# laomao0/BIN

Hardware: AMD Instinct MI355X
Metric: interpolated frames/sec at 1280x720 (higher is better)
Workload: dtype f16x3 (fp16 hi+lo pairs = 22-bit significands, 3 MFMA products, f32 accumulate; fp32-class: 1e-6 vs the fp32 reference); 1 GPU; Adobe240 test_blur 1280x720 inference, batch=1 per GPU (6-frame window padded to 768x1344 by the test.py rule), window-sharded; precision=f16x3, streams=1, pipelined_steps=False, four_call_schedule=False, parity=max-abs <= 2e-5 (f16x3) vs the fp32 reference (tests/)

## Files before the change

bin_amd/_lib.py:

```python
import ctypes as C
import os
from functools import partial

from . import build as _build
from .build import BY_NAME, LIB_PATH

RDN_LAYERS = 66
RDN_MAX_LAYERS, RDN_MAX_CONVS = 192, 7
PLAN_KEEP_ACTS, PLAN_NO_FUSE, PLAN_RDB3, PLAN_FUSED_UPNET, PLAN_FUSED_UPNET_TRAIN = 1, 2, 4, 8, 16
PLAN_UPNET_FOLD = 32
BWD_ACCUMULATE = 1
BWD_SAVED_X3 = 2
BWD_FUSED_UPNET = 4
EPI_PLANES, EPI_SHUFFLE, EPI_FINAL, EPI_FINAL_SUBPIX = 0, 1, 2, 4
PROF_WGRAD = 16
LOSS_CHARBONNIER, LOSS_L1_SUM, LOSS_L2_SUM = 0, 1, 2
RDN_LAYOUT_WORDS, RDN_BWD_LAYOUT_WORDS = 16, 24


class BinConvDesc(C.Structure):
    _fields_ = [("N", C.c_int32), ("H", C.c_int32), ("W", C.c_int32), ("ksize", C.c_int32),
                ("cin_chunks", C.c_int32), ("cout", C.c_int32), ("cout_pad", C.c_int32),
                ("nterms", C.c_int32), ("epilogue", C.c_int32), ("relu", C.c_int32),
                ("x_cpg", C.c_int32), ("x_group_stride", C.c_int64), ("n_images", C.c_int32),
                ("reserved", C.c_int32), ("status", C.c_void_p)]


LOSS_MAX_TERMS = 24
CONV_HALF_LAST_CHUNK = 1
CONV_UPNET_FOLD = 2


class BinLossTerms(C.Structure):
    _fields_ = [("x", C.c_void_p * LOSS_MAX_TERMS), ("y", C.c_void_p * LOSS_MAX_TERMS), ("n_terms", C.c_int32)]


class BinLossGrads(C.Structure):
    _fields_ = [("out", C.c_void_p * LOSS_MAX_TERMS), ("term_a", C.c_int32 * LOSS_MAX_TERMS),
                ("term_b", C.c_int32 * LOSS_MAX_TERMS), ("sign_a", C.c_float * LOSS_MAX_TERMS),
                ("sign_b", C.c_float * LOSS_MAX_TERMS), ("n_out", C.c_int32)]


class BinRdnShape(C.Structure):
# ... 356 lines not shown
```

bin_amd/csrc/binhip_fused.h:

```cpp
#pragma once
#include "binhip_conv_common.h"

struct TailKArgs {
    const _Float16 *x_hi, *x_lo;
    const _Float16 *wc_hi, *wc_lo;
    const _Float16 *wl_hi, *wl_lo;
    const float *bc, *bl;
    _Float16 *y_hi, *y_lo;
    _Float16 *o3_hi, *o3_lo;
    unsigned* flags;
    int N, H, W, tiles_x, tiles_y, wt;
#if BINHIP_TIMELINE
    void* tl;
    unsigned tl_launch, tl_base;
#endif
};

int bh_launch_tail_x3(const TailKArgs& a, hipStream_t s);
```

bin_amd/csrc/binhip_fused_x3.hip:

```cpp
#include "binhip_fused.h"
#include <type_traits>

namespace {

struct TX {
    static constexpr int R = 2, NW = 4, TH = 8, PH = 10, PW = 34;
    static constexpr int PP = (PH * PW * 2 + 63) / 64;
    static constexpr int CWP = 9, LWP = 3;
    static constexpr int PATCH_BYTES = PP * 1024;
    static constexpr int WPL = (CWP + LWP) * 1024;
    static constexpr int WBUF_BYTES = 2 * WPL;
    static constexpr int W_OFF = 2 * PATCH_BYTES;
    static constexpr int LDS_BYTES = W_OFF + 2 * WBUF_BYTES;
    static constexpr int NCHUNK = 12;
    static constexpr int NPJ = (PP + NW - 1) / NW;
    static constexpr int TAILW_OFF = W_OFF;
    static_assert(2 * LDS_BYTES <= 160 * 1024, "two workgroups per CU");
};

__device__ __forceinline__ void tx_issue_patch(const TailKArgs& a, char* smem, int c, int pl, int wave, const unsigned* voff,
                                               const ConvTile& t) {
    __amdgpu_buffer_rsrc_t rs = patch_plane(a, c, pl, t);
    char* lds = smem + pl * TX::PATCH_BYTES;
#pragma unroll
    for (int j = 0; j < TX::NPJ; ++j) {
        const int i = wave + TX::NW * j;
        if (i < TX::PP) __builtin_amdgcn_raw_ptr_buffer_load_lds(rs, (lds_void_t*)(lds + i * 1024), 16, voff[j], 0, 0, 0);
    }
}

__device__ __forceinline__ void tx_issue_weights(const TailKArgs& a, char* smem, int c, int buf, int wave, int lane) {
    __amdgpu_buffer_rsrc_t ch = __builtin_amdgcn_make_buffer_rsrc((void*)(a.wc_hi + (long long)c * (9 * 32 * 16)), 0, 9 * 1024, 0x00020000);
    __amdgpu_buffer_rsrc_t cl = __builtin_amdgcn_make_buffer_rsrc((void*)(a.wc_lo + (long long)c * (9 * 32 * 16)), 0, 9 * 1024, 0x00020000);
    __amdgpu_buffer_rsrc_t lh = __builtin_amdgcn_make_buffer_rsrc((void*)(a.wl_hi + (long long)c * (96 * 16)), 0, 3 * 1024, 0x00020000);
    __amdgpu_buffer_rsrc_t ll = __builtin_amdgcn_make_buffer_rsrc((void*)(a.wl_lo + (long long)c * (96 * 16)), 0, 3 * 1024, 0x00020000);
    char* lds = smem + TX::W_OFF + buf * TX::WBUF_BYTES;
    const unsigned v = (unsigned)(lane * 16);
#pragma unroll
    for (int j = 0; j < 6; ++j) {
        const int i = wave + TX::NW * j;
        const int pl = i >= 12 ? 1 : 0;
        const int k = i - 12 * pl;
        const bool lff = k >= TX::CWP;
        const int t = lff ? k - TX::CWP : k;
        __builtin_amdgcn_raw_ptr_buffer_load_lds(pl ? (lff ? ll : cl) : (lff ? lh : ch), (lds_void_t*)(lds + i * 1024), 16, v,
                                                 t * 1024, 0, 0);
    }
}

__device__ __forceinline__ void tx_issue_tailw(const TailKArgs& a, char* smem, int wave, int lane) {
    __amdgpu_buffer_rsrc_t lh = __builtin_amdgcn_make_buffer_rsrc((void*)(a.wl_hi + (long long)12 * (96 * 16)), 0, 6 * 1024, 0x00020000);
    __amdgpu_buffer_rsrc_t ll = __builtin_amdgcn_make_buffer_rsrc((void*)(a.wl_lo + (long long)12 * (96 * 16)), 0, 6 * 1024, 0x00020000);
    char* lds = smem + TX::TAILW_OFF;
#pragma unroll
    for (int j = 0; j < 3; ++j) {
        const int i = wave + TX::NW * j;
        const int pl = i >= 6 ? 1 : 0;
        __builtin_amdgcn_raw_ptr_buffer_load_lds(pl ? ll : lh, (lds_void_t*)(lds + i * 1024), 16, (unsigned)(lane * 16),
                                                 (i - 6 * pl) * 1024, 0, 0);
    }
}

template <int RES>
__device__ __forceinline__ void tx_add_residual_row(const half8& bc, floatx16 (&accl)[3][TX::R], int r) {
    constexpr int K = RES >> 1, HF = RES & 1;
    union H8 { half8 h; unsigned u[4]; };
    H8 v;
    v.h = bc;
#pragma unroll
    for (int k = 0; k < 2; ++k) {
        auto sw = __builtin_amdgcn_permlane32_swap(v.u[k], v.u[2 + k], false, false);
        v.u[k] = sw[0]; v.u[2 + k] = sw[1];
    }
#pragma unroll
    for (int ge = 0; ge < 2; ++ge)
#pragma unroll
        for (int j = 0; j < 4; ++j) accl[K][r][4 * (2 * HF + ge) + j] += (float)v.h[4 * ge + j];
}

template <bool HI, int RES>
__device__ __forceinline__ void tx_compute(const char* pb, const char* wb, int a_lane_off, int b_lane_off,
                                           floatx16 (&accc)[TX::R], floatx16 (&accl)[3][TX::R], half8 (&carry)[TX::R]) {
    constexpr int R = TX::R;
    constexpr int NSTEP = 12;
    half8 B[2][R + 2];
    half8 Ah[2], Al[2];
    auto load_b = [&](int dx, half8 (&dst)[R + 2]) {
#pragma unroll
        for (int rr = 0; rr < R + 2; ++rr) dst[rr] = ld8(pb + b_lane_off + (rr * TX::PW + dx) * 16);
    };
    auto step_kind = [](int s, bool& lff, int& dx, int& k) {
        if (s < 3) { lff = false; dx = 0; k = s; }
        else if (s < 6) { lff = false; dx = 1; k = s - 3; }
        else if (s < 9) { lff = true; dx = 1; k = s - 6; }
// ... 19 lines not shown
        if constexpr (RES >= 0) {
            if (s == 0) {
#pragma unroll
                for (int r = 0; r < R; ++r) tx_add_residual_row<RES>(carry[r], accl, r);
                __builtin_amdgcn_sched_barrier(0);
            }
        }
        if (!lff) {
            const int set = dx & 1;
            if constexpr (HI) {
#pragma unroll
                for (int r = 0; r < R; ++r)
                    accc[r] = mfma_32x32x16(Al[s & 1], B[set][r + k], accc[r]);
            }
#pragma unroll
            for (int r = 0; r < R; ++r)
                accc[r] = mfma_32x32x16(Ah[s & 1], B[set][r + k], accc[r]);
        } else {
            if constexpr (HI) {
#pragma unroll
                for (int r = 0; r < R; ++r)
                    accl[k][r] = mfma_32x32x16(Al[s & 1], B[1][r + 1], accl[k][r]);
            }
#pragma unroll
            for (int r = 0; r < R; ++r)
                accl[k][r] = mfma_32x32x16(Ah[s & 1], B[1][r + 1], accl[k][r]);
        }
        __builtin_amdgcn_sched_barrier(0);
    }
#pragma unroll
    for (int r = 0; r < R; ++r) carry[r] = B[1][r + 1];
}

__global__ void __launch_bounds__(256) __attribute__((amdgpu_waves_per_eu(2, 2)))
rdb_tail_x3_kernel(const TailKArgs a, const float* __restrict__ bias_c, const float* __restrict__ bias_l) {
    extern __shared__ __attribute__((aligned(16))) char smem[];
    BH_TL_DECL;
    BH_TL_BEGIN();
    const int tid = threadIdx.x;
    const int lane = tid & 63;
    const int wave = __builtin_amdgcn_readfirstlane(tid >> 6);
    const int n = lane & 31, kg = lane >> 5;

    const ConvTile t = tile_decode<TX::TH>(a, 1);
    const int img = t.img, tx0 = t.tx0, ty0 = t.ty0;
    const int H = a.H, W = a.W;
    const long long plane_elems = t.plane_elems;
    unsigned voff[TX::NPJ];
    patch_offsets<TX, 1>(voff, t, H, W, wave, lane);

    floatx16 accc[TX::R];
    floatx16 accl[3][TX::R];
#pragma unroll
    for (int r = 0; r < TX::R; ++r)
#pragma unroll
        for (int e = 0; e < 16; ++e) {
            accc[r][e] = 0.f;
            accl[0][r][e] = 0.f; accl[1][r][e] = 0.f; accl[2][r][e] = 0.f;
        }
    const int a_lane_off = weight_lane_off(n, kg);
    const int b_lane_off = patch_lane_off<TX>(n, kg, wave * TX::R);

    __builtin_amdgcn_s_setprio(2);
    tx_issue_weights(a, smem, 0, 0, wave, lane);
    tx_issue_patch(a, smem, 0, 0, wave, voff, t);
    half8 carry[TX::R];
    auto chunk = [&](const int c, auto res_hi, auto res_lo) __attribute__((always_inline)) {
        constexpr int RH = decltype(res_hi)::value, RL = decltype(res_lo)::value;
        const char* wb = smem + TX::W_OFF + (c & 1) * TX::WBUF_BYTES;
        wait_vmcnt<0>();
        __builtin_amdgcn_s_barrier();
        __builtin_amdgcn_sched_barrier(0);
#if BINHIP_TIMELINE
        if (c == 0) BH_TL_STAMP(1);
#endif
        tx_issue_patch(a, smem, c, 1, wave, voff, t);
        if (c + 1 < TX::NCHUNK) tx_issue_weights(a, smem, c + 1, (c + 1) & 1, wave, lane);
        else tx_issue_tailw(a, smem, wave, lane);
        tx_compute<true, RH>(smem, wb, a_lane_off, b_lane_off, accc, accl, carry);
        wait_vmcnt<0>();
        __builtin_amdgcn_s_barrier();
        __builtin_amdgcn_sched_barrier(0);
        if (c + 1 < TX::NCHUNK) tx_issue_patch(a, smem, c + 1, 0, wave, voff, t);
        tx_compute<false, RL>(smem + TX::PATCH_BYTES, wb, a_lane_off, b_lane_off, accc, accl, carry);
    };
    using std::integral_constant;
    chunk(0, integral_constant<int, -1>{}, integral_constant<int, 0>{});
    chunk(1, integral_constant<int, 0>{}, integral_constant<int, 1>{});
    chunk(2, integral_constant<int, 1>{}, integral_constant<int, 2>{});
    chunk(3, integral_constant<int, 2>{}, integral_constant<int, 3>{});
    chunk(4, integral_constant<int, 3>{}, integral_constant<int, 4>{});
    chunk(5, integral_constant<int, 4>{}, integral_constant<int, 5>{});
    chunk(6, integral_constant<int, 5>{}, integral_constant<int, -1>{});
    for (int c = 7; c < TX::NCHUNK; ++c) chunk(c, integral_constant<int, -1>{}, integral_constant<int, -1>{});
    wait_vmcnt<0>();
    __builtin_amdgcn_s_barrier();
    __builtin_amdgcn_sched_barrier(0);

    __builtin_amdgcn_s_setprio(0);
    const int gx = tx0 + n;
    union H4 { half4 h; unsigned u[2]; };
    union H8 { half8 h; unsigned u[4]; };
    unsigned sat = 0;
    half8 Bh[2][TX::R], Bl[2][TX::R];
#pragma unroll
    for (int r = 0; r < TX::R; ++r) {
        const int gy = ty0 + wave * TX::R + r;
        const bool ok = (gy < H) && (gx < W);
#pragma unroll
        for (int gp = 0; gp < 2; ++gp) {
            H4 hv[2], lv[2];
#pragma unroll
            for (int ge = 0; ge < 2; ++ge) {
                const int g = 2 * gp + ge;
                float b8[8];
#pragma unroll
                for (int j = 0; j < 8; ++j) b8[j] = bias_c[8 * g + j];
                const float v[4] = {accc[r][4 * g + 0] + (kg ? b8[4] : b8[0]), accc[r][4 * g + 1] + (kg ? b8[5] : b8[1]),
                                    accc[r][4 * g + 2] + (kg ? b8[6] : b8[2]), accc[r][4 * g + 3] + (kg ? b8[7] : b8[3])};
                split_pair(v[0], v[1], sat, hv[ge].u[0], lv[ge].u[0], true);
                split_pair(v[2], v[3], sat, hv[ge].u[1], lv[ge].u[1], true);
            }
#pragma unroll
            for (int k = 0; k < 2; ++k) {
                auto sw = __builtin_amdgcn_permlane32_swap(hv[0].u[k], hv[1].u[k], false, false);
                hv[0].u[k] = sw[0]; hv[1].u[k] = sw[1];
                auto sl = __builtin_amdgcn_permlane32_swap(lv[0].u[k], lv[1].u[k], false, false);
                lv[0].u[k] = sl[0]; lv[1].u[k] = sl[1];
            }
            H8 fh, fl;
            fh.u[0] = hv[0].u[0]; fh.u[1] = hv[0].u[1]; fh.u[2] = hv[1].u[0]; fh.u[3] = hv[1].u[1];
            fl.u[0] = lv[0].u[0]; fl.u[1] = lv[0].u[1]; fl.u[2] = lv[1].u[0]; fl.u[3] = lv[1].u[1];
            Bh[gp][r] = fh.h;
            Bl[gp][r] = fl.h;
            if (a.o3_hi && ok) {
                const long long o = (long long)gp * plane_elems + ((((long long)img * H + gy) * W + gx) << 4) + kg * 8;
                *reinterpret_cast<uint4*>(a.o3_hi + o) = make_uint4(fh.u[0], fh.u[1], fh.u[2], fh.u[3]);
                *reinterpret_cast<uint4*>(a.o3_lo + o) = make_uint4(fl.u[0], fl.u[1], fl.u[2], fl.u[3]);
            }
        }
    }

    const char* tailw = smem + TX::TAILW_OFF;
#pragma unroll
    for (int t = 0; t < 2; ++t) {
#pragma unroll
        for (int mt = 0; mt < 3; ++mt) {
            const int off = (t * 96 + mt * 32) * 32 + a_lane_off;
            const half8 Ah = ld8(tailw + off);
            const half8 Al = ld8(tailw + 6 * 1024 + off);
#pragma unroll
            for (int r = 0; r < TX::R; ++r) {
                accl[mt][r] = mfma_32x32x16(Al, Bh[t][r], accl[mt][r]);
                accl[mt][r] = mfma_32x32x16(Ah, Bh[t][r], accl[mt][r]);
                accl[mt][r] = mfma_32x32x16(Ah, Bl[t][r], accl[mt][r]);
            }
        }
    }
    if (a.flags && __builtin_amdgcn_ballot_w64(sat != 0) != 0 && lane == 0) atomicOr(a.flags, BINHIP_FLAG_SATURATED);
    BH_TL_STAMP(2);

    ConvKArgs e;
    e.bias = a.bl; e.y_hi = a.y_hi; e.y_lo = a.y_lo;
    e.r_hi = e.r_lo = e.r2_hi = e.r2_lo = e.m_hi = nullptr;
    e.flags = a.flags;
    e.N = a.N; e.H = H; e.W = W;
    e.relu = 0; e.has_res = 0; e.cout = 96; e.wt = a.wt;
    e.och_limit = 6; e.res_chunks = 0; e.mask_from = 0; e.y_cpg = 0; e.y_cpg_inv = 0; e.y_group_stride = 0; e.y_unshuf = 0;
    conv_epilogue<3, TX::R, 3, BINHIP_EPI_PLANES, false>(e, bias_l, accl, img, ty0 + wave * TX::R, tx0, 0, true, n, kg, plane_elems);
    BH_TL_FINISH(a, blockIdx.x);
}

}

int bh_launch_tail_x3(const TailKArgs& a0, hipStream_t s) {
    static std::atomic<unsigned long long> lds_set{0};
    if (int rc = bh_set_max_lds(&rdb_tail_x3_kernel, TX::LDS_BYTES, lds_set)) return rc;
    TailKArgs a = a0;
    const unsigned grid = set_tiles<TX>(a);
#if BINHIP_TIMELINE
    a.tl = bh_tl_reserve(grid, &a.tl_base);
    a.tl_launch = (2u << 24) | (g_bh_tl_serial.fetch_add(1) & 0xFFFFFFu);
#endif
    rdb_tail_x3_kernel<<<dim3(grid), dim3(256), TX::LDS_BYTES, s>>>(a, a.bc, a.bl);
    BH_CHECK_LAUNCH();
    return 0;
}
```

bin_amd/csrc/binhip_plan.hip:

```cpp
#include "binhip_conv_common.h"

namespace {

struct Shp {
    int G0, D, C, G;
    int c0, cg, cb;
    int L;
    bool stage4;
};
bool resolve_shape(const BinRdnShape* s, Shp* o) {
    Shp h;
    const bool dflt = !s || (s->G0 == 0 && s->D == 0 && s->C == 0 && s->G == 0);
    h.G0 = dflt ? 96 : s->G0; h.D = dflt ? 12 : s->D; h.C = dflt ? 4 : s->C; h.G = dflt ? 32 : s->G;
    if (h.G0 < 32 || h.G0 > 256 || h.G0 % 32 || h.G < 32 || h.G > 128 || h.G % 32) return false;
    if (h.C < 1 || h.C > BINHIP_RDN_MAX_CONVS || h.D < 1 || h.D > 20) return false;
    h.c0 = h.G0 / 16; h.cg = h.G / 16; h.cb = h.c0 + h.C * h.cg;
    h.L = 2 + h.D * (h.C + 1) + 4;
    if (h.L > BINHIP_RDN_MAX_LAYERS) return false;
    h.stage4 = (h.G0 == 96 && h.C == 4 && h.G == 32);
    *o = h;
    return true;
}
inline int layer_conv(const Shp& sh, int d, int c) { return 2 + d * (sh.C + 1) + c; }

bool frames_ok(int N, int H, int W, int n_inputs) {
    return N > 0 && H > 0 && W > 0 && !(H & 1) && !(W & 1) && (n_inputs == 2 || n_inputs == 3 || n_inputs == 5) &&
           (long long)N * H * W < (1ll << 26);
}

struct Planes {
    int64_t off = -1, size = 0;
    bool present() const { return off >= 0; }
    Planes sub(int64_t elems) const { return {off + elems, size}; }
// ... 41 lines not shown
    int x_cpg = 0;
    int64_t x_group_stride = 0;
    Planes y, res;
    int reserved = 0;
};

}

extern "C" {

size_t binhip_rdn_workspace_bytes(int N, int H, int W, int n_inputs, int nterms, const BinRdnShape* shape) {
    Shp sh;
    if (!frames_ok(N, H, W, n_inputs) || !resolve_shape(shape, &sh)) return 0;
    return (size_t)make_ws(N, H, W, n_inputs, nterms, sh).total * 2 + 256;
}

int binhip_rdn_workspace_layout(int N, int H, int W, int n_inputs, int nterms, const BinRdnShape* shape, int64_t* out, int n_out) {
    if (!out || n_out < BINHIP_RDN_LAYOUT_WORDS) return BINHIP_E_ARG;
    Shp sh;
    if (!frames_ok(N, H, W, n_inputs) || !resolve_shape(shape, &sh)) return BINHIP_E_SHAPE;
    const Ws w = make_ws(N, H, W, n_inputs, nterms, sh);
    const Planes t[6] = {w.x0, w.f1, w.blk, w.g0, w.g1, w.u};
    out[0] = w.P; out[1] = w.PF; out[2] = w.kc0; out[15] = nterms == 3 ? 1 : 0;
    for (int i = 0; i < 6; ++i) { out[3 + 2 * i] = t[i].off; out[4 + 2 * i] = t[i].size; }
    return 0;
}

int binhip_rdn_forward(const BinRdnPlan* p, const float* const* inputs, float* out, void* workspace, size_t workspace_bytes, void* stream) {
    if (!p || !inputs || !out || !workspace) return BINHIP_E_ARG;
    const int N = p->N, H = p->H, W = p->W, nin = p->n_inputs, nt = p->nterms;
    if (!frames_ok(N, H, W, nin)) return BINHIP_E_SHAPE;
    if (nt != 1 && nt != 3) return BINHIP_E_ARG;
    if (p->reserved & ~(BINHIP_PLAN_KEEP_ACTS | BINHIP_PLAN_NO_FUSE | BINHIP_PLAN_RDB3 | BINHIP_PLAN_FUSED_UPNET | BINHIP_PLAN_FUSED_UPNET_TRAIN |
                        BINHIP_PLAN_UPNET_FOLD)) return BINHIP_E_ARG;
    if ((p->reserved & BINHIP_PLAN_UPNET_FOLD) && (nt != 3 || (p->reserved & BINHIP_PLAN_KEEP_ACTS) || !(p->reserved & BINHIP_PLAN_FUSED_UPNET)))
        return BINHIP_E_ARG;
    Shp sh;
    if (!resolve_shape(&p->shape, &sh)) return BINHIP_E_SHAPE;
    const size_t need = binhip_rdn_workspace_bytes(N, H, W, nin, nt, &p->shape);
    if (workspace_bytes < need) return BINHIP_E_WORKSPACE;
    for (int i = 0; i < nin; ++i) if (!inputs[i]) return BINHIP_E_ARG;
    for (int i = 0; i < sh.L; ++i) if (!p->w_hi[i] || !p->bias[i] || (nt == 3 && !p->w_lo[i])) return BINHIP_E_ARG;

    hipStream_t s = (hipStream_t)stream;
    const Ws w = make_ws(N, H, W, nin, nt, sh);
    const int h = H / 2, ww = W / 2;
    const Bind A(workspace, nt == 3);

    int rc = binhip_pack_inputs(inputs, nin, N, H, W, A.hi(w.x0), A.lo(w.x0), p->status, stream);
    if (rc) return rc;

    auto mk = [&](const Conv& l) -> BhConvCall {
        BhConvCall c;
        c.d.N = N; c.d.H = l.H ? l.H : h; c.d.W = l.W ? l.W : ww; c.d.ksize = l.ks; c.d.cin_chunks = l.cin_chunks; c.d.cout = l.cout;
        c.d.cout_pad = l.cout_pad ? l.cout_pad : l.cout; c.d.nterms = nt; c.d.epilogue = l.epi; c.d.relu = l.relu;
        c.d.x_cpg = l.x_cpg; c.d.x_group_stride = l.x_group_stride; c.d.status = p->status; c.d.reserved = l.reserved;
        if (l.ks == 1 && l.epi == BINHIP_EPI_PLANES && c.d.W > 32 && c.d.W % 32 == 0) { c.d.H *= c.d.W / 32; c.d.W = 32; }
        if (l.layer == 0 && l.ks == 5 && (12 * nin) % 16 >= 1 && (12 * nin) % 16 <= 8) c.d.reserved = BINHIP_CONV_HALF_LAST_CHUNK;
        c.x_hi = A.hi(l.x); c.x_lo = A.lo(l.x);
        c.w_hi = p->w_hi[l.layer]; c.w_lo = p->w_lo[l.layer]; c.bias = p->bias[l.layer];
        c.r_hi = A.hi(l.res); c.r_lo = A.lo(l.res);
        c.y_hi = A.hi(l.y); c.y_lo = A.lo(l.y);
        c.status = p->status; c.prof = p->profiler;
        if (l.epi == BINHIP_EPI_FINAL || l.epi == BINHIP_EPI_FINAL_SUBPIX) {
            c.y_f32 = out; c.d.n_images = nin;
            for (int i = 0; i < nin; ++i) c.images[i] = inputs[i];
        }
        return c;
    };
    auto conv = [&](const Conv& l) -> int { return bh_launch_conv(mk(l), s); };
    const bool rdb3 = (p->reserved & BINHIP_PLAN_RDB3) && nt == 3 && sh.stage4;
    unsigned* sync_words = (unsigned*)(A.base + w.sync);
    const int cus = binhip_device_cus();
    if (rdb3) {
        hipError_t me = hipMemsetAsync(sync_words, 0, (size_t)(32 + 2 * (size_t)w.tiles) * 4, s);
        if (me != hipSuccess) return (int)me;
    }
    const int64_t P = w.P;
    const int G0 = sh.G0, G = sh.G, C = sh.C, D = sh.D, c0 = sh.c0, cg = sh.cg, cb = sh.cb;
    if ((rc = conv({.layer = 0, .ks = 5, .cin_chunks = w.kc0, .cout = G0, .x = w.x0, .y = w.f1}))) return rc;
    if ((rc = conv({.layer = 1, .cin_chunks = c0, .cout = G0, .x = w.f1, .y = w.blk}))) return rc;
    for (int d = 0; d < D; ++d) {
        const Planes b = w.blk.sub((int64_t)d * cb * P), b_next = b.sub(cb * P);
        auto dense = [&](int c) -> Conv {
            return {.layer = layer_conv(sh, d, c), .cin_chunks = c0 + cg * c, .cout = G, .relu = 1, .x = b, .y = b.sub((c0 + cg * c) * P)};
        };
        const bool fuse = sh.stage4 && !(p->reserved & BINHIP_PLAN_NO_FUSE);
        bool done3 = false;
        if (rdb3 && fuse) {
            ConvKArgs ka[3];
            bool ok3 = true;
            for (int c = 0; c < 3 && ok3; ++c) {
                if ((rc = bh_prepare_conv(mk(dense(c)), &ka[c]))) return rc;
                ok3 = ok3 && ka[c].wt;
            }
            if (ok3) {
                rc = bh_launch_rdb3_x3(ka, sync_words + 32, (unsigned)(d + 1), cus, s);
                if (rc == 0) done3 = true;
                else if (rc != BINHIP_E_SHAPE) return rc;
            }
        }
        for (int c = 0; c < (fuse ? C - 1 : C) && !done3; ++c) if ((rc = conv(dense(c)))) return rc;
        if (fuse) {
            const int L3 = layer_conv(sh, d, 3), LF = layer_conv(sh, d, 4);
            if ((rc = binhip_rdb_tail_fwd(N, h, ww, nt, A.hi(b), A.lo(b), p->w_hi[L3], p->w_lo[L3], p->bias[L3], p->w_hi[LF], p->w_lo[LF], p->bias[LF],
                                          A.hi(b_next), A.lo(b_next), (p->reserved & BINHIP_PLAN_KEEP_ACTS) ? 1 : 0, p->status, stream)))
                return rc;
        } else if ((rc = conv({.layer = layer_conv(sh, d, C), .ks = 1, .cin_chunks = cb, .cout = G0, .x = b, .y = b_next, .res = b})))
            return rc;
    }
    const int LG = sh.L - 4;
    if ((rc = conv({.layer = LG, .ks = 1, .cin_chunks = D * c0, .cout = G0, .x = w.blk.sub(cb * P), .x_cpg = c0, .x_group_stride = cb * P, .y = w.g0})))
        return rc;
    if ((rc = conv({.layer = LG + 1, .cin_chunks = c0, .cout = G0, .x = w.g0, .y = w.g1, .res = w.f1}))) return rc;
    const bool fused_up = (p->reserved & BINHIP_PLAN_FUSED_UPNET) &&
                          (!(p->reserved & BINHIP_PLAN_KEEP_ACTS) || (p->reserved & BINHIP_PLAN_FUSED_UPNET_TRAIN)) &&
                          sh.L + 1 < BINHIP_RDN_MAX_LAYERS && p->w_hi[sh.L] && (nt == 1 || p->w_lo[sh.L]) && p->bias[sh.L] &&
                          p->w_hi[sh.L + 1] && p->bias[sh.L + 1];
    const bool fold = (p->reserved & BINHIP_PLAN_UPNET_FOLD) != 0;
    if (fused_up) {
        if ((rc = conv({.layer = sh.L, .ks = 5, .cin_chunks = c0, .cout = 12, .cout_pad = 32, .epi = BINHIP_EPI_FINAL_SUBPIX, .x = w.g1,
                        .reserved = fold ? BINHIP_CONV_UPNET_FOLD : 0})))
            return rc;
        return bh_launch_upnet_ring(A.hi(w.g1), A.lo(w.g1), (const float*)p->w_hi[sh.L + 1], p->bias[sh.L + 1], out, inputs, nin, N, h, ww,
                                    G0, s);
    }
    if ((rc = conv({.layer = LG + 2, .cin_chunks = c0, .cout = 256, .epi = BINHIP_EPI_SHUFFLE, .x = w.g1, .y = w.u}))) return rc;
    return conv({.layer = LG + 3, .cin_chunks = 4, .cout = 3, .cout_pad = 32, .epi = BINHIP_EPI_FINAL, .H = H, .W = W, .x = w.u});
}

}

namespace {

struct Bws {
    int64_t P, PF;
    int kc0, gx0_chunks;
    Planes gout, gu, guu, gg1, gg0, gf1, gy, gcat, gcat2, gx0;
    size_t wg_bytes, sc_off_bytes, wg_off_bytes, total_bytes;
};

Bws make_bws(int N, int H, int W, int nin, int nt, const Shp& sh) {
    Bws b;
    const int h = H / 2, w = W / 2;
    b.P = (int64_t)N * h * w * 16; b.PF = (int64_t)N * H * W * 16;
// ... 232 lines not shown
```

bin_amd/rdn_plan.py:

```python
import ctypes as C

import torch

from . import _lib as L
from .ops import ConvWeights, DgradWeights, RdbGatherWeights, _ptr, _stream, _need_cuda, on_device, relayout_batch, status_word

STAGE4_SHAPE = (96, 12, 4, 32)


def check_shape(shape):
    G0, D, C, G = (int(v) for v in shape)
    if G0 % 32 or not 32 <= G0 <= 256 or G % 32 or not 32 <= G <= 128 or not 1 <= C <= L.RDN_MAX_CONVS or not 1 <= D <= 20 \
            or 2 + D * (C + 1) + 4 > L.RDN_MAX_LAYERS:
        raise NotImplementedError(
            f"bin_amd RDN: unsupported configuration G0={G0}, D={D}, C={C}, G={G} (built: G0 and G multiples of 32 with "
            f"32 <= G0 <= 256, G <= 128; 1 <= C <= {L.RDN_MAX_CONVS}; 1 <= D <= 20)")
    return G0, D, C, G


def c_shape(shape):
    s = L.BinRdnShape()
    s.G0, s.D, s.C, s.G = shape
    return s

# ... 285 lines not shown

def workspace(nbytes, device, key="fwd"):
    stream = torch.cuda.current_stream(device)
    if torch.cuda.is_current_stream_capturing():
        return torch.empty(nbytes, dtype=torch.uint8, device=device)
    key = (device.type, device.index, stream.cuda_stream, key)
    ws = _workspaces.get(key)
    if ws is None or ws.numel() < nbytes:
        ws = torch.empty(nbytes, dtype=torch.uint8, device=device)
        _workspaces[key] = ws
        while len(_workspaces) > WORKSPACE_CACHE_ENTRIES:
            _workspaces.popitem(last=False)
    _workspaces.move_to_end(key)
    return ws


def release_workspaces(stream=None):
    if stream is None:
        _workspaces.clear()
        return
    for k in [k for k in _workspaces if k[2] == stream.cuda_stream and k[1] == stream.device.index]:
        del _workspaces[k]


import os as _os


def default_plan_flags():
    flags = L.PLAN_RDB3 if _os.environ.get("BIN_AMD_RDB3", "0") == "1" else 0
    if _os.environ.get("BIN_AMD_FUSED_UPNET", "1") != "0":
        flags |= L.PLAN_FUSED_UPNET
        if _os.environ.get("BIN_AMD_UPNET_FOLD", "1") != "0":
            flags |= L.PLAN_UPNET_FOLD
    return flags


def rdn_forward(weights, inputs, out=None, ws=None, flags=0, profiler=None):
    _need_cuda(*inputs)
    with on_device(inputs[0]):
        return _rdn_forward(weights, inputs, out, ws, flags, profiler)


def _rdn_forward(weights, inputs, out, ws, flags, profiler):
    inputs = [t.contiguous().float() for t in inputs]
    n, c, h, w = inputs[0].shape
    assert c == 3 and len(inputs) == weights.n_inputs
    lib = L.lib()
    plan = L.BinRdnPlan()
    plan.N, plan.H, plan.W, plan.n_inputs, plan.nterms = n, h, w, weights.n_inputs, weights.nterms
    plan.reserved = int(flags or 0)
    plan.status = status_word(inputs[0].device).data_ptr()
    plan.profiler = profiler if profiler else None
    fused, fold = None, False
    if plan.reserved & L.PLAN_FUSED_UPNET:
        if plan.reserved & L.PLAN_FUSED_UPNET_TRAIN:
            fused = weights.ensure_fused_upnet(train=True)
        elif not (plan.reserved & L.PLAN_KEEP_ACTS):
            fused = weights.ensure_fused_upnet()
            fold = bool(plan.reserved & L.PLAN_UPNET_FOLD) and fused is not None and weights.fused_fold is not None
    if not fold:
        plan.reserved &= ~L.PLAN_UPNET_FOLD
    weights.fill_plan(plan, fused, fold)
    nbytes = lib.binhip_rdn_workspace_bytes(n, h, w, weights.n_inputs, weights.nterms, C.byref(plan.shape))
    if nbytes == 0:
        raise RuntimeError(f"bin_amd: unsupported RDN shape N={n} H={h} W={w} (H, W must be even)")
    if ws is None:
        ws = workspace(nbytes, inputs[0].device)
    if out is None:
        out = torch.empty((n, 3, h, w), dtype=torch.float32, device=inputs[0].device)
    arr = (C.c_void_p * len(inputs))(*[t.data_ptr() for t in inputs])
    L.check(lib.binhip_rdn_forward(C.byref(plan), arr, _ptr(out), _ptr(ws), ws.numel(), _stream()), "rdn_forward")
    return out
```

include/binhip.h:

```cpp
#ifndef BINHIP_H
#define BINHIP_H

#include <stddef.h>
#include <stdint.h>

#ifdef __cplusplus
extern "C" {
#endif

#define BINHIP_API __attribute__((visibility("default")))

#define BINHIP_VERSION 622
#define BINHIP_ABI_EXPORTS 51

#define BINHIP_E_ARG      (-1)
#define BINHIP_E_SHAPE    (-2)
#define BINHIP_E_WORKSPACE (-3)

#define BINHIP_STATUS_SATURATED 1u
#define BINHIP_STATUS_SYNC_TIMEOUT 2u

#define BINHIP_EPI_PLANES  0
#define BINHIP_EPI_SHUFFLE 1
#define BINHIP_EPI_FINAL   2
// ... 102 lines not shown
BINHIP_API int binhip_pixel_loss_fwd(int kind, const float* x, const float* y, int64_t numel, float eps,
                          float* partials, float* loss, void* stream);
BINHIP_API int binhip_pixel_loss_bwd(int kind, const float* x, const float* y, int64_t numel, float eps,
                          const float* gloss, float* gx, float* gy, void* stream);

#define BINHIP_LOSS_MAX_TERMS 24
typedef struct {
    const float* x[BINHIP_LOSS_MAX_TERMS];
    const float* y[BINHIP_LOSS_MAX_TERMS];
    int32_t n_terms;
} BinLossTerms;
BINHIP_API int binhip_multi_loss_fwd(int kind, const BinLossTerms* t, int64_t numel, float eps, float* partials, float* terms,
                          float* loss, void* stream);
typedef struct {
    float* out[BINHIP_LOSS_MAX_TERMS];
    int32_t term_a[BINHIP_LOSS_MAX_TERMS], term_b[BINHIP_LOSS_MAX_TERMS];
    float sign_a[BINHIP_LOSS_MAX_TERMS], sign_b[BINHIP_LOSS_MAX_TERMS];
    int32_t n_out;
} BinLossGrads;
BINHIP_API int binhip_multi_loss_bwd(int kind, const BinLossTerms* t, int64_t numel, float eps, const float* gloss,
                          const BinLossGrads* g, void* stream);

BINHIP_API int binhip_rdb_tail_fwd(int N, int H, int W, int nterms, const void* blk_hi, const void* blk_lo,
                        const void* wc_hi, const void* wc_lo, const float* bias_c,
                        const void* wl_hi, const void* wl_lo, const float* bias_l,
                        void* y_hi, void* y_lo, int store_o3, void* status, void* stream);

#define BINHIP_PLAN_KEEP_ACTS 1
#define BINHIP_PLAN_NO_FUSE   2
#define BINHIP_PLAN_RDB3      4
#define BINHIP_PLAN_FUSED_UPNET 8
#define BINHIP_PLAN_FUSED_UPNET_TRAIN 16
#define BINHIP_PLAN_UPNET_FOLD 32
typedef struct BinRdnPlan {
    int32_t N, H, W;
    int32_t n_inputs;
    int32_t nterms;
    int32_t reserved;
    BinRdnShape shape;
    const void* w_hi[BINHIP_RDN_MAX_LAYERS];
    const void* w_lo[BINHIP_RDN_MAX_LAYERS];
    const float* bias[BINHIP_RDN_MAX_LAYERS];
    void* status;
    struct BinhipProfiler* profiler;
} BinRdnPlan;

BINHIP_API size_t binhip_rdn_workspace_bytes(int N, int H, int W, int n_inputs, int nterms, const BinRdnShape* shape );
#define BINHIP_RDN_LAYOUT_WORDS 16
BINHIP_API int binhip_rdn_workspace_layout(int N, int H, int W, int n_inputs, int nterms, const BinRdnShape* shape,
                                int64_t* out, int n_out);
BINHIP_API int binhip_rdn_forward(const BinRdnPlan* plan, const float* const* inputs , float* out ,
                       void* workspace, size_t workspace_bytes, void* stream);

BINHIP_API size_t binhip_wgrad_workspace_bytes(int ksize, int N, int H, int W, int cin_chunks, int cout);
BINHIP_API int binhip_conv2d_bwd_weight(const BinConvDesc* d, const void* x_hi, const void* x_lo,
                             const void* gy_hi, const void* gy_lo, const float* inv_scale,
                             void* workspace, size_t workspace_bytes, float* dw_oihw, float* dbias,
                             int cin, int shuffle_perm, int accumulate, void* stream);

BINHIP_API int binhip_grad_scale(const float* g, int64_t numel, float target, float* partials, float* scale_out,
                      void* stream);
BINHIP_API int binhip_nchw_to_planes_scaled(const float* x, int N, int C, int H, int W, const float* scale,
                                 void* y_hi, void* y_lo, void* status, void* stream);
BINHIP_API int binhip_unshuffle_planes(const void* x_hi, const void* x_lo, int N, int H, int W, int nchunks,
                            void* y_hi, void* y_lo, void* stream);
BINHIP_API int binhip_unpack_input_grads(const void* gx0_hi, const void* gx0_lo, const float* gout,
// ... 64 lines not shown
```

Before: 16.82 interpolated frames/s.

## Fuse global feature fusion 1x1 conv into the last RDB tail kernel

For the last dense block, the tail kernel now also computes the global feature fusion 1x1 convolution. It streams the earlier blocks' outputs through a three-stage LDS ring and folds in the last block's output straight from registers, so that output is never written out and the separate GFF conv launch is skipped. This saves a full-resolution write and re-read of the final block output plus one kernel launch. In exchange the tail kernel gets longer and heavier on registers, and its per-tile LDS ring may pipeline less well than the standalone conv.

```diff
diff --git a/bin_amd/_lib.py b/bin_amd/_lib.py
--- a/bin_amd/_lib.py
+++ b/bin_amd/_lib.py
@@ -9,6 +9,7 @@
 RDN_MAX_LAYERS, RDN_MAX_CONVS = 192, 7
 PLAN_KEEP_ACTS, PLAN_NO_FUSE, PLAN_RDB3, PLAN_FUSED_UPNET, PLAN_FUSED_UPNET_TRAIN = 1, 2, 4, 8, 16
 PLAN_UPNET_FOLD = 32
+PLAN_GFF_IN_TAIL = 64
 BWD_ACCUMULATE = 1
 BWD_SAVED_X3 = 2
 BWD_FUSED_UPNET = 4
diff --git a/bin_amd/csrc/binhip_fused.h b/bin_amd/csrc/binhip_fused.h
--- a/bin_amd/csrc/binhip_fused.h
+++ b/bin_amd/csrc/binhip_fused.h
@@ -10,6 +10,12 @@
     _Float16 *o3_hi, *o3_lo;
     unsigned* flags;
     int N, H, W, tiles_x, tiles_y, wt;
+    const _Float16 *g_hi = nullptr, *g_lo = nullptr;
+    const float* g_bias = nullptr;
+    const _Float16 *gx_hi = nullptr, *gx_lo = nullptr;
+    long long gx_group_stride = 0;
+    int gx_groups = 0;
+    _Float16 *gy_hi = nullptr, *gy_lo = nullptr;
 #if BINHIP_TIMELINE
     void* tl;
     unsigned tl_launch, tl_base;
diff --git a/bin_amd/csrc/binhip_fused_x3.hip b/bin_amd/csrc/binhip_fused_x3.hip
--- a/bin_amd/csrc/binhip_fused_x3.hip
+++ b/bin_amd/csrc/binhip_fused_x3.hip
@@ -18,6 +18,21 @@
     static_assert(2 * LDS_BYTES <= 160 * 1024, "two workgroups per CU");
 };
 
+struct GX {
+    static constexpr int NW = TX::NW, PH = TX::TH, PW = 32;
+    static constexpr int PP = PH * PW * 2 / 64, NPJ = PP / NW;
+    static constexpr int XPL = PP * 1024, GPL = 3 * 1024;
+    static constexpr int G_OFF = 2 * XPL;
+    static constexpr int STAGE_BYTES = G_OFF + 2 * GPL;
+    static constexpr int NBUF = 3;
+    static constexpr int PS_X = 2 * NPJ + 2, PS_G = 2;
+    static constexpr int DUMMY_OFF = TX::W_OFF + STAGE_BYTES;
+    __host__ __device__ static constexpr int buf_off(int b) { return b == 0 ? 0 : (b == 1 ? TX::W_OFF + TX::WBUF_BYTES : TX::W_OFF); }
+    static_assert(STAGE_BYTES <= 2 * TX::PATCH_BYTES && STAGE_BYTES <= TX::WBUF_BYTES && DUMMY_OFF + 1024 <= TX::W_OFF + TX::WBUF_BYTES,
+                  "the three stages and the dummy piece fit the tail's carve-up");
+    static_assert(NPJ * NW == PP, "whole pieces per wave");
+};
+
 __device__ __forceinline__ void tx_issue_patch(const TailKArgs& a, char* smem, int c, int pl, int wave, const unsigned* voff,
                                                const ConvTile& t) {
     __amdgpu_buffer_rsrc_t rs = patch_plane(a, c, pl, t);
@@ -60,6 +75,47 @@
                                                  (i - 6 * pl) * 1024, 0, 0);
     }
 }
+
+__device__ __forceinline__ void tx_issue_gff(const TailKArgs& a, char* smem, int st, int nstream, int buf, int wave, int lane,
+                                             const unsigned* gvoff, const ConvTile& t) {
+    char* lds = smem + GX::buf_off(buf);
+    if (st < nstream) {
+        const long long coff = (long long)(st / 6) * a.gx_group_stride + (long long)(st % 6) * t.plane_elems;
+#pragma unroll
+        for (int pl = 0; pl < 2; ++pl) {
+            __amdgpu_buffer_rsrc_t rs = __builtin_amdgcn_make_buffer_rsrc((void*)((pl ? a.gx_lo : a.gx_hi) + coff), 0, t.plane_bytes, 0x00020000);
+#pragma unroll
+            for (int j = 0; j < GX::NPJ; ++j)
+                __builtin_amdgcn_raw_ptr_buffer_load_lds(rs, (lds_void_t*)(lds + pl * GX::XPL + (wave + GX::NW * j) * 1024), 16, gvoff[j], 0, 0, 0);
+        }
+    }
+    __amdgpu_buffer_rsrc_t gh = __builtin_amdgcn_make_buffer_rsrc((void*)(a.g_hi + (long long)st * (96 * 16)), 0, GX::GPL, 0x00020000);
+    __amdgpu_buffer_rsrc_t gl = __builtin_amdgcn_make_buffer_rsrc((void*)(a.g_lo + (long long)st * (96 * 16)), 0, GX::GPL, 0x00020000);
+#pragma unroll
+    for (int j = 0; j < 2; ++j) {
+        const int i = wave + GX::NW * j;
+        const bool real = i < 6;
+        __builtin_amdgcn_raw_ptr_buffer_load_lds(i >= 3 ? gl : gh, (lds_void_t*)(real ? lds + GX::G_OFF + i * 1024 : smem + GX::DUMMY_OFF), 16,
+                                                 real ? (unsigned)(lane * 16) : 0x80000000u, real ? (i % 3) * 1024 : 0, 0, 0);
+    }
+}
+
+template <int R0, int NR>
+__device__ __forceinline__ void tx_gff_step(const char* gw, int a_lane_off, const half8 (&Bh)[NR], const half8 (&Bl)[NR],
+                                            floatx16 (&gff)[3][TX::R]) {
+#pragma unroll
+    for (int mt = 0; mt < 3; ++mt) {
+        const half8 Ah = ld8(gw + mt * 1024 + a_lane_off);
+        const half8 Al = ld8(gw + GX::GPL + mt * 1024 + a_lane_off);
+#pragma unroll
+        for (int r = 0; r < NR; ++r) {
+            gff[mt][R0 + r] = mfma_32x32x16(Al, Bh[r], gff[mt][R0 + r]);
+            gff[mt][R0 + r] = mfma_32x32x16(Ah, Bl[r], gff[mt][R0 + r]);
+            gff[mt][R0 + r] = mfma_32x32x16(Ah, Bh[r], gff[mt][R0 + r]);
+        }
+    }
+}
+
 
 template <int RES>
 __device__ __forceinline__ void tx_add_residual_row(const half8& bc, floatx16 (&accl)[3][TX::R], int r) {
@@ -145,8 +201,9 @@
     for (int r = 0; r < R; ++r) carry[r] = B[1][r + 1];
 }
 
+template <bool GFF>
 __global__ void __launch_bounds__(256) __attribute__((amdgpu_waves_per_eu(2, 2)))
-rdb_tail_x3_kernel(const TailKArgs a, const float* __restrict__ bias_c, const float* __restrict__ bias_l) {
+rdb_tail_x3_kernel(const TailKArgs a, const float* __restrict__ bias_c, const float* __restrict__ bias_l, const float* __restrict__ bias_g) {
     extern __shared__ __attribute__((aligned(16))) char smem[];
     BH_TL_DECL;
     BH_TL_BEGIN();
@@ -210,11 +267,46 @@
     __builtin_amdgcn_s_barrier();
     __builtin_amdgcn_sched_barrier(0);
 
+    const int g_nstream = GFF ? 6 * a.gx_groups : 0, g_nst = g_nstream + 6;
+    unsigned gvoff[GX::NPJ];
+    if constexpr (GFF) {
+        patch_offsets<GX, 0>(gvoff, t, H, W, wave, lane);
+        tx_issue_gff(a, smem, 0, g_nstream, 0, wave, lane, gvoff, t);
+        tx_issue_gff(a, smem, 1, g_nstream, 1, wave, lane, gvoff, t);
+    }
+
     __builtin_amdgcn_s_setprio(0);
     const int gx = tx0 + n;
-    union H4 { half4 h; unsigned u[2]; };
     union H8 { half8 h; unsigned u[4]; };
     unsigned sat = 0;
+    auto acc_to_frag = [&](const floatx16& acc, const float* __restrict__ bias, int co0, int gp, auto relu, half8& fh, half8& fl)
+        __attribute__((always_inline)) {
+        union H4 { half4 h; unsigned u[2]; };
+        H4 hv[2], lv[2];
+#pragma unroll
+        for (int ge = 0; ge < 2; ++ge) {
+            const int g = 2 * gp + ge;
+            float b8[8];
+#pragma unroll
+            for (int j = 0; j < 8; ++j) b8[j] = bias[co0 + 8 * g + j];
+            const float v[4] = {acc[4 * g + 0] + (kg ? b8[4] : b8[0]), acc[4 * g + 1] + (kg ? b8[5] : b8[1]),
+                                acc[4 * g + 2] + (kg ? b8[6] : b8[2]), acc[4 * g + 3] + (kg ? b8[7] : b8[3])};
+            split_pair(v[0], v[1], sat, hv[ge].u[0], lv[ge].u[0], decltype(relu)::value);
+            split_pair(v[2], v[3], sat, hv[ge].u[1], lv[ge].u[1], decltype(relu)::value);
+        }
+#pragma unroll
+        for (int k = 0; k < 2; ++k) {
+            auto sw = __builtin_amdgcn_permlane32_swap(hv[0].u[k], hv[1].u[k], false, false);
+            hv[0].u[k] = sw[0]; hv[1].u[k] = sw[1];
+            auto sl = __builtin_amdgcn_permlane32_swap(lv[0].u[k], lv[1].u[k], false, false);
+            lv[0].u[k] = sl[0]; lv[1].u[k] = sl[1];
+        }
+        H8 h, l;
+        h.u[0] = hv[0].u[0]; h.u[1] = hv[0].u[1]; h.u[2] = hv[1].u[0]; h.u[3] = hv[1].u[1];
+        l.u[0] = lv[0].u[0]; l.u[1] = lv[0].u[1]; l.u[2] = lv[1].u[0]; l.u[3] = lv[1].u[1];
+        fh = h.h;
+        fl = l.h;
+    };
     half8 Bh[2][TX::R], Bl[2][TX::R];
 #pragma unroll
     for (int r = 0; r < TX::R; ++r) {
@@ -222,28 +314,8 @@
         const bool ok = (gy < H) && (gx < W);
 #pragma unroll
         for (int gp = 0; gp < 2; ++gp) {
-            H4 hv[2], lv[2];
-#pragma unroll
-            for (int ge = 0; ge < 2; ++ge) {
-                const int g = 2 * gp + ge;
-                float b8[8];
-#pragma unroll
-                for (int j = 0; j < 8; ++j) b8[j] = bias_c[8 * g + j];
-                const float v[4] = {accc[r][4 * g + 0] + (kg ? b8[4] : b8[0]), accc[r][4 * g + 1] + (kg ? b8[5] : b8[1]),
-                                    accc[r][4 * g + 2] + (kg ? b8[6] : b8[2]), accc[r][4 * g + 3] + (kg ? b8[7] : b8[3])};
-                split_pair(v[0], v[1], sat, hv[ge].u[0], lv[ge].u[0], true);
-                split_pair(v[2], v[3], sat, hv[ge].u[1], lv[ge].u[1], true);
-            }
-#pragma unroll
-            for (int k = 0; k < 2; ++k) {
-                auto sw = __builtin_amdgcn_permlane32_swap(hv[0].u[k], hv[1].u[k], false, false);
-                hv[0].u[k] = sw[0]; hv[1].u[k] = sw[1];
-                auto sl = __builtin_amdgcn_permlane32_swap(lv[0].u[k], lv[1].u[k], false, false);
-                lv[0].u[k] = sl[0]; lv[1].u[k] = sl[1];
-            }
             H8 fh, fl;
-            fh.u[0] = hv[0].u[0]; fh.u[1] = hv[0].u[1]; fh.u[2] = hv[1].u[0]; fh.u[3] = hv[1].u[1];
-            fl.u[0] = lv[0].u[0]; fl.u[1] = lv[0].u[1]; fl.u[2] = lv[1].u[0]; fl.u[3] = lv[1].u[1];
+            acc_to_frag(accc[r], bias_c, 0, gp, std::true_type{}, fh.h, fl.h);
             Bh[gp][r] = fh.h;
             Bl[gp][r] = fl.h;
             if (a.o3_hi && ok) {
@@ -270,32 +342,97 @@
             }
         }
     }
+    auto store_planes = [&](const float* bias_arg, const float* __restrict__ bias, _Float16* y_hi, _Float16* y_lo, floatx16 (&acc)[3][TX::R])
+        __attribute__((always_inline)) {
+        ConvKArgs e;
+        e.bias = bias_arg; e.y_hi = y_hi; e.y_lo = y_lo;
+        e.r_hi = e.r_lo = e.r2_hi = e.r2_lo = e.m_hi = nullptr;
+        e.flags = a.flags;
+        e.N = a.N; e.H = H; e.W = W;
+        e.relu = 0; e.has_res = 0; e.cout = 96; e.wt = a.wt;
+        e.och_limit = 6; e.res_chunks = 0; e.mask_from = 0; e.y_cpg = 0; e.y_cpg_inv = 0; e.y_group_stride = 0; e.y_unshuf = 0;
+        conv_epilogue<3, TX::R, 3, BINHIP_EPI_PLANES, false>(e, bias, acc, img, ty0 + wave * TX::R, tx0, 0, true, n, kg, plane_elems);
+    };
+    floatx16 gff[3][TX::R];
+    if constexpr (GFF) {
+        asm volatile("" : "+v"(sat));
+        __builtin_amdgcn_s_setprio(2);
+#pragma unroll
+        for (int mt = 0; mt < 3; ++mt)
+#pragma unroll
+            for (int r = 0; r < TX::R; ++r)
+#pragma unroll
+                for (int e = 0; e < 16; ++e) gff[mt][r][e] = 0.f;
+        const int gb_lane_off = patch_lane_off<GX>(n, kg, wave * TX::R);
+        int cur = 0;
+        auto ring_step = [&](int st) __attribute__((always_inline)) {
+            if (st + 1 >= g_nst) wait_vmcnt<0>();
+            else if (st + 1 < g_nstream) wait_vmcnt<GX::PS_X>();
+            else wait_vmcnt<GX::PS_G>();
+            __builtin_amdgcn_s_barrier();
+            __builtin_amdgcn_sched_barrier(0);
+            if (st + 2 < g_nst) tx_issue_gff(a, smem, st + 2, g_nstream, cur == 0 ? 2 : cur - 1, wave, lane, gvoff, t);
+        };
+        for (int st = 0; st < g_nstream; ++st) {
+            ring_step(st);
+            const char* sb = smem + GX::buf_off(cur);
+            half8 Xh[TX::R], Xl[TX::R];
+#pragma unroll
+            for (int r = 0; r < TX::R; ++r) {
+                Xh[r] = ld8(sb + gb_lane_off + r * GX::PW * 16);
+                Xl[r] = ld8(sb + GX::XPL + gb_lane_off + r * GX::PW * 16);
+            }
+            tx_gff_step<0, TX::R>(sb + GX::G_OFF, a_lane_off, Xh, Xl, gff);
+            cur = cur + 1 == GX::NBUF ? 0 : cur + 1;
+        }
+#pragma unroll
+        for (int ch = 0; ch < 6; ++ch) {
+            ring_step(g_nstream + ch);
+            const char* gw = smem + GX::buf_off(cur) + GX::G_OFF;
+            auto row = [&](auto rc) __attribute__((always_inline)) {
+                constexpr int r = decltype(rc)::value;
+                H8 fh, fl;
+                acc_to_frag(accl[ch >> 1][r], bias_l, 32 * (ch >> 1), ch & 1, std::false_type{}, fh.h, fl.h);
+                const bool ok = (ty0 + wave * TX::R + r < H) && (gx < W);
+#pragma unroll
+                for (int k = 0; k < 4; ++k) { fh.u[k] = ok ? fh.u[k] : 0u; fl.u[k] = ok ? fl.u[k] : 0u; }
+                const half8 Yh[1] = {fh.h}, Yl[1] = {fl.h};
+                asm volatile("" : "+v"(sat));
+                tx_gff_step<r, 1>(gw, a_lane_off, Yh, Yl, gff);
+                __builtin_amdgcn_sched_barrier(0);
+            };
+            row(integral_constant<int, 0>{});
+            row(integral_constant<int, 1>{});
+            cur = cur + 1 == GX::NBUF ? 0 : cur + 1;
+        }
+        __builtin_amdgcn_s_setprio(0);
+    }
     if (a.flags && __builtin_amdgcn_ballot_w64(sat != 0) != 0 && lane == 0) atomicOr(a.flags, BINHIP_FLAG_SATURATED);
     BH_TL_STAMP(2);
-
-    ConvKArgs e;
-    e.bias = a.bl; e.y_hi = a.y_hi; e.y_lo = a.y_lo;
-    e.r_hi = e.r_lo = e.r2_hi = e.r2_lo = e.m_hi = nullptr;
-    e.flags = a.flags;
-    e.N = a.N; e.H = H; e.W = W;
-    e.relu = 0; e.has_res = 0; e.cout = 96; e.wt = a.wt;
-    e.och_limit = 6; e.res_chunks = 0; e.mask_from = 0; e.y_cpg = 0; e.y_cpg_inv = 0; e.y_group_stride = 0; e.y_unshuf = 0;
-    conv_epilogue<3, TX::R, 3, BINHIP_EPI_PLANES, false>(e, bias_l, accl, img, ty0 + wave * TX::R, tx0, 0, true, n, kg, plane_elems);
+    if constexpr (GFF) store_planes(a.g_bias, bias_g, a.gy_hi, a.gy_lo, gff);
+    else store_planes(a.bl, bias_l, a.y_hi, a.y_lo, accl);
     BH_TL_FINISH(a, blockIdx.x);
 }
 
 }
 
 int bh_launch_tail_x3(const TailKArgs& a0, hipStream_t s) {
-    static std::atomic<unsigned long long> lds_set{0};
-    if (int rc = bh_set_max_lds(&rdb_tail_x3_kernel, TX::LDS_BYTES, lds_set)) return rc;
+    static std::atomic<unsigned long long> lds_set{0}, lds_set_gff{0};
+    const bool gff = a0.g_hi != nullptr;
+    if (gff && (!a0.g_lo || !a0.g_bias || !a0.gy_hi || !a0.gy_lo || a0.gx_groups < 0 || a0.gx_group_stride < 0 ||
+                (a0.gx_groups > 0 && (!a0.gx_hi || !a0.gx_lo)) || a0.o3_hi))
+        return BINHIP_E_ARG;
+    if (int rc = gff ? bh_set_max_lds(&rdb_tail_x3_kernel<true>, TX::LDS_BYTES, lds_set_gff)
+                     : bh_set_max_lds(&rdb_tail_x3_kernel<false>, TX::LDS_BYTES, lds_set))
+        return rc;
     TailKArgs a = a0;
     const unsigned grid = set_tiles<TX>(a);
 #if BINHIP_TIMELINE
     a.tl = bh_tl_reserve(grid, &a.tl_base);
     a.tl_launch = (2u << 24) | (g_bh_tl_serial.fetch_add(1) & 0xFFFFFFu);
 #endif
-    rdb_tail_x3_kernel<<<dim3(grid), dim3(256), TX::LDS_BYTES, s>>>(a, a.bc, a.bl);
+    if (gff) rdb_tail_x3_kernel<true><<<dim3(grid), dim3(256), TX::LDS_BYTES, s>>>(a, a.bc, a.bl, a.g_bias);
+    else rdb_tail_x3_kernel<false><<<dim3(grid), dim3(256), TX::LDS_BYTES, s>>>(a, a.bc, a.bl, a.bl);
     BH_CHECK_LAUNCH();
     return 0;
 }
diff --git a/bin_amd/csrc/binhip_plan.hip b/bin_amd/csrc/binhip_plan.hip
--- a/bin_amd/csrc/binhip_plan.hip
+++ b/bin_amd/csrc/binhip_plan.hip
@@ -1,4 +1,6 @@
-#include "binhip_conv_common.h"
+#include "binhip_fused.h"
+
+int bh_launch_tail_x3(const TailKArgs& a, hipStream_t s) __attribute__((weak));
 
 namespace {
 
@@ -106,11 +108,15 @@
     if (!frames_ok(N, H, W, nin)) return BINHIP_E_SHAPE;
     if (nt != 1 && nt != 3) return BINHIP_E_ARG;
     if (p->reserved & ~(BINHIP_PLAN_KEEP_ACTS | BINHIP_PLAN_NO_FUSE | BINHIP_PLAN_RDB3 | BINHIP_PLAN_FUSED_UPNET | BINHIP_PLAN_FUSED_UPNET_TRAIN |
-                        BINHIP_PLAN_UPNET_FOLD)) return BINHIP_E_ARG;
+                        BINHIP_PLAN_UPNET_FOLD | BINHIP_PLAN_GFF_IN_TAIL)) return BINHIP_E_ARG;
     if ((p->reserved & BINHIP_PLAN_UPNET_FOLD) && (nt != 3 || (p->reserved & BINHIP_PLAN_KEEP_ACTS) || !(p->reserved & BINHIP_PLAN_FUSED_UPNET)))
         return BINHIP_E_ARG;
+    const bool gff_tail = (p->reserved & BINHIP_PLAN_GFF_IN_TAIL) != 0;
+    if (gff_tail && (nt != 3 || (p->reserved & (BINHIP_PLAN_KEEP_ACTS | BINHIP_PLAN_NO_FUSE))))
+        return BINHIP_E_ARG;
     Shp sh;
     if (!resolve_shape(&p->shape, &sh)) return BINHIP_E_SHAPE;
+    if (gff_tail && (!sh.stage4 || !bh_launch_tail_x3)) return BINHIP_E_ARG;
     const size_t need = binhip_rdn_workspace_bytes(N, H, W, nin, nt, &p->shape);
     if (workspace_bytes < need) return BINHIP_E_WORKSPACE;
     for (int i = 0; i < nin; ++i) if (!inputs[i]) return BINHIP_E_ARG;
@@ -177,14 +183,32 @@
         for (int c = 0; c < (fuse ? C - 1 : C) && !done3; ++c) if ((rc = conv(dense(c)))) return rc;
         if (fuse) {
             const int L3 = layer_conv(sh, d, 3), LF = layer_conv(sh, d, 4);
-            if ((rc = binhip_rdb_tail_fwd(N, h, ww, nt, A.hi(b), A.lo(b), p->w_hi[L3], p->w_lo[L3], p->bias[L3], p->w_hi[LF], p->w_lo[LF], p->bias[LF],
+            if (gff_tail && d == D - 1) {
+                const int LG0 = sh.L - 4;
+                TailKArgs a;
+                a.x_hi = (const _Float16*)A.hi(b); a.x_lo = (const _Float16*)A.lo(b);
+                a.wc_hi = (const _Float16*)p->w_hi[L3]; a.wc_lo = (const _Float16*)p->w_lo[L3];
+                a.wl_hi = (const _Float16*)p->w_hi[LF]; a.wl_lo = (const _Float16*)p->w_lo[LF];
+                a.bc = p->bias[L3]; a.bl = p->bias[LF];
+                a.y_hi = a.y_lo = a.o3_hi = a.o3_lo = nullptr;
+                a.flags = (unsigned*)p->status;
+                a.N = N; a.H = h; a.W = ww; a.tiles_x = a.tiles_y = 0;
+                a.wt = (6 * P * 2 < (1ll << 32) - 64) ? 1 : 0;
+                a.g_hi = (const _Float16*)p->w_hi[LG0]; a.g_lo = (const _Float16*)p->w_lo[LG0]; a.g_bias = p->bias[LG0];
+                const Planes first_out = w.blk.sub(cb * P);
+                a.gx_hi = (const _Float16*)A.hi(first_out); a.gx_lo = (const _Float16*)A.lo(first_out);
+                a.gx_group_stride = cb * P; a.gx_groups = D - 1;
+                a.gy_hi = (_Float16*)A.hi(w.g0); a.gy_lo = (_Float16*)A.lo(w.g0);
+                if ((rc = bh_launch_tail_x3(a, s))) return rc;
+            } else if ((rc = binhip_rdb_tail_fwd(N, h, ww, nt, A.hi(b), A.lo(b), p->w_hi[L3], p->w_lo[L3], p->bias[L3], p->w_hi[LF], p->w_lo[LF], p->bias[LF],
                                           A.hi(b_next), A.lo(b_next), (p->reserved & BINHIP_PLAN_KEEP_ACTS) ? 1 : 0, p->status, stream)))
                 return rc;
         } else if ((rc = conv({.layer = layer_conv(sh, d, C), .ks = 1, .cin_chunks = cb, .cout = G0, .x = b, .y = b_next, .res = b})))
             return rc;
     }
     const int LG = sh.L - 4;
-    if ((rc = conv({.layer = LG, .ks = 1, .cin_chunks = D * c0, .cout = G0, .x = w.blk.sub(cb * P), .x_cpg = c0, .x_group_stride = cb * P, .y = w.g0})))
+    if (!gff_tail &&
+        (rc = conv({.layer = LG, .ks = 1, .cin_chunks = D * c0, .cout = G0, .x = w.blk.sub(cb * P), .x_cpg = c0, .x_group_stride = cb * P, .y = w.g0})))
         return rc;
     if ((rc = conv({.layer = LG + 1, .cin_chunks = c0, .cout = G0, .x = w.g0, .y = w.g1, .res = w.f1}))) return rc;
     const bool fused_up = (p->reserved & BINHIP_PLAN_FUSED_UPNET) &&
diff --git a/bin_amd/rdn_plan.py b/bin_amd/rdn_plan.py
--- a/bin_amd/rdn_plan.py
+++ b/bin_amd/rdn_plan.py
@@ -341,7 +341,14 @@
         flags |= L.PLAN_FUSED_UPNET
         if _os.environ.get("BIN_AMD_UPNET_FOLD", "1") != "0":
             flags |= L.PLAN_UPNET_FOLD
+    if _os.environ.get("BIN_AMD_GFF_IN_TAIL", "1") != "0":
+        flags |= L.PLAN_GFF_IN_TAIL
     return flags
+
+
+def gff_in_tail_legal(flags, nterms, shape):
+    G0, _, C, G = shape
+    return nterms == 3 and not (flags & (L.PLAN_KEEP_ACTS | L.PLAN_NO_FUSE)) and (G0, C, G) == (96, 4, 32)
 
 
 def rdn_forward(weights, inputs, out=None, ws=None, flags=0, profiler=None):
@@ -369,6 +376,8 @@
             fold = bool(plan.reserved & L.PLAN_UPNET_FOLD) and fused is not None and weights.fused_fold is not None
     if not fold:
         plan.reserved &= ~L.PLAN_UPNET_FOLD
+    if not gff_in_tail_legal(plan.reserved, weights.nterms, weights.shape):
+        plan.reserved &= ~L.PLAN_GFF_IN_TAIL
     weights.fill_plan(plan, fused, fold)
     nbytes = lib.binhip_rdn_workspace_bytes(n, h, w, weights.n_inputs, weights.nterms, C.byref(plan.shape))
     if nbytes == 0:
diff --git a/include/binhip.h b/include/binhip.h
--- a/include/binhip.h
+++ b/include/binhip.h
@@ -158,6 +158,7 @@
 #define BINHIP_PLAN_FUSED_UPNET 8
 #define BINHIP_PLAN_FUSED_UPNET_TRAIN 16
 #define BINHIP_PLAN_UPNET_FOLD 32
+#define BINHIP_PLAN_GFF_IN_TAIL 64
 typedef struct BinRdnPlan {
     int32_t N, H, W;
     int32_t n_inputs;
```

After: 17.04 interpolated frames/s, median of 6. 1.3% higher.
